# Christovis/astrild

Measured on AMD Instinct MI355X. Metric: particles/sec CIC+3D-FFT P(k) on 1024^3 grid, higher is better.
Workload: dtype f32

## Files before the change

astrild_amd/csrc/fft_tile.hip:

```cpp
#include "ast_common.h"
#include "paint_tile_geom.h"
#include <algorithm>
#include <cmath>
#include <cstring>
#include <mutex>
#include <vector>

namespace {

__device__ constexpr float kCos32[16] = {
    1.0f, 0.9807852804032304f, 0.9238795325112867f, 0.8314696123025452f, 0.7071067811865476f,
    0.5555702330196023f, 0.38268343236508984f, 0.19509032201612833f, 0.0f, -0.1950903220161282f,
    -0.3826834323650897f, -0.555570233019602f, -0.7071067811865475f, -0.8314696123025453f,
    -0.9238795325112867f, -0.9807852804032304f};
__device__ constexpr float kSin32[16] = {
    0.0f, 0.19509032201612825f, 0.3826834323650898f, 0.5555702330196022f, 0.7071067811865475f,
    0.8314696123025452f, 0.9238795325112867f, 0.9807852804032304f, 1.0f, 0.9807852804032304f,
    0.9238795325112867f, 0.8314696123025455f, 0.7071067811865476f, 0.5555702330196022f,
    0.3826834323650899f, 0.1950903220161286f};

#ifndef FFT_NT
#define FFT_NT 3
#endif
typedef float f2v __attribute__((ext_vector_type(2)));
template <bool NT>
__device__ inline float2 ld_stream(const float2* p) {
    if (NT && (FFT_NT & 1)) { const f2v v = __builtin_nontemporal_load(reinterpret_cast<const f2v*>(p)); return make_float2(v.x, v.y); }
    return *p;
}
template <bool NT>
__device__ inline void st_stream(float2* p, float2 v) {
    if (NT && (FFT_NT & 2)) __builtin_nontemporal_store(f2v{v.x, v.y}, reinterpret_cast<f2v*>(p));
    else *p = v;
}
typedef float cf2 __attribute__((ext_vector_type(2)));
__device__ inline cf2 to_cf(float2 a) { return cf2{a.x, a.y}; }
__device__ inline float2 from_cf(cf2 a) { return make_float2(a.x, a.y); }
__device__ inline cf2 cmul_cf(cf2 a, cf2 w) {
    return __builtin_elementwise_fma(a.yy, cf2{-w.y, w.x}, a.xx * w);
}
__device__ inline float2 cmul(float2 a, float2 w) { return from_cf(cmul_cf(to_cf(a), to_cf(w))); }

constexpr int bitrev(int v, int bits) {
    int r = 0;
    for (int i = 0; i < bits; ++i) r |= ((v >> i) & 1) << (bits - 1 - i);
    return r;
}
constexpr int ilog2(int v) { return v <= 1 ? 0 : 1 + ilog2(v / 2); }

template <int R>
__device__ inline void fft_reg(float2 (&vv)[R]) {
    cf2 v[R];
#pragma unroll
    for (int i = 0; i < R; ++i) v[i] = to_cf(vv[i]);
#pragma unroll
    for (int h = R / 2; h >= 1; h /= 2) {
#pragma unroll
        for (int blk = 0; blk < R; blk += 2 * h) {
#pragma unroll
            for (int j = 0; j < h; ++j) {
                const cf2 a = v[blk + j], b = v[blk + j + h];
                v[blk + j] = a + b;
                const cf2 d = a - b;
                const int t = j * (16 / h);
                if (t == 0) v[blk + j + h] = d;
                else if (t == 8) v[blk + j + h] = d.yx * cf2{1.0f, -1.0f};
                else v[blk + j + h] = cmul_cf(d, cf2{kCos32[t], -kSin32[t]});
            }
        }
    }
#pragma unroll
    for (int i = 0; i < R; ++i) vv[i] = from_cf(v[i]);
}

__device__ inline int tile_isqrt(int v) {
    return (int)__builtin_amdgcn_sqrtf((float)v + 0.5f);
}

__global__ void tile_isqrt_table_kernel(int* out, int count) {
    for (int v = blockIdx.x * blockDim.x + threadIdx.x; v < count; v += gridDim.x * blockDim.x) out[v] = tile_isqrt(v);
}

struct ShellMask { const float2* src; long long lo2, hi2; int ky0 = 0; int pass = 0;
                   size_t src_elem_stride = 0, src_batch_stride = 0; };

constexpr int SHELL_BATCH = 8;
#ifndef C2C_XCD_MODE
#define C2C_XCD_MODE 2
#endif
struct ShellBatch { int count = 0; float2* work[SHELL_BATCH]; long long lo2[SHELL_BATCH], hi2[SHELL_BATCH]; };
struct C2RBatch { int count = 0; const float2* in[SHELL_BATCH]; float* out[SHELL_BATCH]; int kmax[SHELL_BATCH]; };

struct DiscEntry { int offb; unsigned S, cumS, lohi; };
struct PackDst { float2* out = nullptr; unsigned c1_log2 = 0; unsigned nbatch = 0; float2* self_out = nullptr; unsigned self_part = ~0u; unsigned pitch = 0;
                 const DiscEntry* disc = nullptr; const unsigned short* gk = nullptr; unsigned part = 0;
                 unsigned xmajor = 0; };

template <int R1, int R2, int C, bool POWER, bool INV = false, int PACK = 0>
__global__ void __launch_bounds__(C * (R1 > R2 ? R1 : R2))
__attribute__((amdgpu_waves_per_eu((POWER || C > 16) && R1 * R2 >= 1024 ? 4 : 1, (POWER || C > 16) && R1 * R2 >= 1024 ? 4 : 8)))
strided_c2c_kernel(float2* __restrict__ data, const float2* __restrict__ tw_g, size_t elem_stride,
                   size_t ncols, size_t batch_stride, unsigned tiles_per_batch, float scale,
                   double* __restrict__ partial, const unsigned* __restrict__ edge_fall, ShellMask mask = ShellMask{nullptr, 0, 0},
                   PackDst pack = PackDst{}, ShellBatch sb = ShellBatch{}) {
    constexpr int N = R1 * R2;
    constexpr int NT = C * (R1 > R2 ? R1 : R2);
    constexpr int NB = N / 2 - 1;
    constexpr bool SPLIT = (POWER || C > 16) && R1 == R2 && N * C * sizeof(float2) > 64 * 1024;
    constexpr int YN = SPLIT ? N / 2 : N;
    extern __shared__ float2 lds[];
    float2* Y = lds;
    float2* tw = lds + YN * C;
    double* shell = reinterpret_cast<double*>(lds + YN * C + N);
    unsigned tile = blockIdx.x % tiles_per_batch, b = blockIdx.x / tiles_per_batch;
#if C2C_XCD_MODE
    if ((INV || C2C_XCD_MODE == 2) && (gridDim.x / tiles_per_batch) % 8u == 0u) {
        const unsigned xcd = blockIdx.x & 7u, slot = blockIdx.x >> 3;
        b = (slot / tiles_per_batch) * 8u + xcd;
        tile = slot % tiles_per_batch;
    }
#endif
    const size_t c0 = (size_t)tile * C;
    if (INV && sb.count > 0) {
        data = sb.work[blockIdx.y];
        mask.lo2 = sb.lo2[blockIdx.y];
        mask.hi2 = sb.hi2[blockIdx.y];
    }
    if (INV && mask.hi2 > 0) {
        const long long kb = (long long)((int)b > N / 2 ? (int)b - N : (int)b);
        const long long r2 = (long long)(c0 * c0) + (mask.pass == 0 ? kb * kb : 0);
        if (r2 >= mask.hi2) return;
    }
    const float2* disc_base = nullptr;
    unsigned disc_S = 0;
    int disc_ky = 0;
    if (!INV && POWER && pack.disc != nullptr) {
        const unsigned subb = b % R1, gk = pack.gk[pack.part * (pack.nbatch / R1) + b / R1];
        const DiscEntry e = pack.disc[(size_t)tile * R2 + gk];
        const unsigned lo = e.lohi & 255u, hi = (e.lohi >> 8) & 255u;
        if (subb - lo >= hi - lo) {
            for (int i = threadIdx.x; i < NB; i += NT) partial[((size_t)b * tiles_per_batch + tile) * NB + i] = 0.0;
            return;
        }
        disc_ky = (int)(gk * R1 + subb);
        if (pack.xmajor) {
            disc_base = data + ((long long)e.offb + (long long)(subb * 16u)) * (long long)pack.xmajor;
            disc_S = 16u;
        } else {
            disc_base = data + ((long long)e.offb + (long long)(subb * 16u));
            disc_S = e.S;
        }
    } else if (!INV && POWER && mask.hi2 > 0) {
        const long long kyi = (long long)b + mask.ky0, ky = kyi > N / 2 ? kyi - N : kyi;
        if (ky * ky + (long long)(c0 * c0) > mask.hi2) {
            for (int i = threadIdx.x; i < NB; i += NT) partial[((size_t)b * tiles_per_batch + tile) * NB + i] = 0.0;
            return;
        }
    }
    for (int i = threadIdx.x; i < N; i += NT) tw[i] = tw_g[i];
    if (POWER)
        for (int i = threadIdx.x; i <= NB; i += NT) shell[i] = 0.0;
    const int c = threadIdx.x % C, sub = threadIdx.x / C;
    const bool col_ok = (unsigned)c0 + (unsigned)c < (unsigned)ncols;
    float2 u[R2];
    {
        const bool task1 = sub < R2;
        float2 v[R1];
        const bool own = INV && mask.src != nullptr && mask.src_elem_stride != 0;
        size_t es_in = own ? mask.src_elem_stride : elem_stride;
        const float2* ubase = (INV && mask.src ? mask.src : data) + (size_t)b * (own ? mask.src_batch_stride : batch_stride);
        const int lsub = task1 ? sub : R2 - 1;
        uint32_t voff = (uint32_t)lsub * (uint32_t)es_in + min((uint32_t)c0 + (uint32_t)c, (uint32_t)ncols - 1u);
        if (POWER && !INV && disc_base != nullptr) {
            es_in = disc_S;
            ubase = disc_base;
            voff = (uint32_t)lsub * disc_S + (uint32_t)c;
        }
        if (INV && mask.hi2 > 0 && mask.pass == 1) {
            const long long c02 = (long long)(c0 * c0);
#pragma unroll
            for (int n1 = 0; n1 < R1; ++n1) {
                const int row = n1 * R2 + lsub;
                const long long ky = row > N / 2 ? row - N : row;
                v[n1] = make_float2(0.f, 0.f);
                if (ky * ky + c02 < mask.hi2) v[n1] = (ubase + (size_t)(n1 * R2) * es_in)[voff];
            }
        } else if (INV && mask.hi2 > 0) {
            const long long kyb = (long long)((int)b > N / 2 ? (int)b - N : (int)b);
            const long long r2yz = kyb * kyb + (long long)(c0 * c0);
#pragma unroll
            for (int n1 = 0; n1 < R1; ++n1) {
                const int lo = n1 * R2, hi = lo + R2 - 1;
                const long long kxmin = hi <= N / 2 ? lo : (lo >= N / 2 ? N - hi : 0);
                v[n1] = make_float2(0.f, 0.f);
                if (kxmin * kxmin + r2yz < mask.hi2) v[n1] = (ubase + (size_t)(n1 * R2) * es_in)[voff];
            }
        } else {
#pragma unroll
            for (int n1 = 0; n1 < R1; ++n1) v[n1] = ld_stream<(!INV && N >= 1024)>(ubase + (size_t)(n1 * R2) * es_in + voff);
        }
        if (INV) {
            if (mask.hi2 > 0 && mask.pass == 0) {
                const long long kz = (long long)min(c0 + c, ncols - 1), ky = (long long)((int)b > N / 2 ? (int)b - N : (int)b);
                const long long m2yz = ky * ky + kz * kz;
#pragma unroll
                for (int n1 = 0; n1 < R1; ++n1) {
                    const int row = n1 * R2 + lsub;
                    const long long kx = row > N / 2 ? row - N : row, m2 = kx * kx + m2yz;
                    if (m2 < mask.lo2 || m2 >= mask.hi2) v[n1] = make_float2(0.f, 0.f);
                }
            }
#pragma unroll
            for (int n1 = 0; n1 < R1; ++n1) v[n1].y = -v[n1].y;
        }
        fft_reg<R1>(v);
        __syncthreads();
        if (!SPLIT) {
            if (task1) {
#pragma unroll
                for (int k1 = 0; k1 < R1; ++k1) {
                    float2 y = v[bitrev(k1, ilog2(R1))];
                    if (k1 != 0) y = cmul(y, tw[sub * k1]);
                    Y[(sub * R1 + k1) * C + c] = y;
                }
            }
            __syncthreads();
            if (sub < R1) {
#pragma unroll
                for (int n2 = 0; n2 < R2; ++n2) u[n2] = Y[(n2 * R1 + sub) * C + c];
            }
        } else {
            constexpr int H = R2 / 2;
#pragma unroll
            for (int half = 0; half < 2; ++half) {
                if (sub / H == half) {
#pragma unroll
                    for (int k1 = 0; k1 < R1; ++k1) {
                        float2 y = v[bitrev(k1, ilog2(R1))];
                        if (k1 != 0) y = cmul(y, tw[sub * k1]);
                        Y[((sub - half * H) * R1 + k1) * C + c] = y;
                    }
                }
                __syncthreads();
#pragma unroll
                for (int nh = 0; nh < H; ++nh) u[half * H + nh] = Y[(nh * R1 + sub) * C + c];
                if (half == 0) __syncthreads();
            }
        }
    }
    if (sub < R1) {
        fft_reg<R2>(u);
        int tid_s = (int)threadIdx.x;
        if (C > 16) asm volatile("" : "+v"(tid_s));
        const int cs = C > 16 ? tid_s % C : c;
        const bool ok_s = C > 16 ? (unsigned)c0 + (unsigned)cs < (unsigned)ncols : col_ok;
        if (PACK == 2 && !POWER) {
            static_assert(PACK != 2 || C == 16, "the disc layout's tiles are 16 columns");
            const int4 ev = reinterpret_cast<const int4*>(pack.disc + (size_t)tile * R2)[threadIdx.x % R2];
#pragma unroll
            for (int k2 = 0; k2 < R2; ++k2) {
                float2 x = u[bitrev(k2, ilog2(R2))];
                x.x *= scale;
                x.y *= scale;
                const int offb = __builtin_amdgcn_readlane(ev.x, k2);
                const unsigned S = (unsigned)__builtin_amdgcn_readlane(ev.y, k2), cumS = (unsigned)__builtin_amdgcn_readlane(ev.z, k2);
                const unsigned lohi = (unsigned)__builtin_amdgcn_readlane(ev.w, k2);
                const unsigned lo = lohi & 255u, hi = (lohi >> 8) & 255u, part = lohi >> 16;
                if (pack.xmajor) {
                    float2* const ub = pack.self_out + ((long long)offb * (long long)pack.xmajor + (long long)(b * 16u));
                    if ((unsigned)sub - lo < hi - lo)
                        st_stream<(N >= 1024)>(ub + ((uint32_t)sub * 16u * pack.xmajor + (uint32_t)(threadIdx.x & 15u)), x);
                    continue;
                }
                float2* const ub = (part == pack.self_part ? pack.self_out : pack.out + (size_t)pack.nbatch * cumS)
                                   + ((size_t)b * S + (long long)offb);
                if ((unsigned)sub - lo < hi - lo) st_stream<(N >= 1024)>(ub + threadIdx.x, x);
            }
        } else if (ok_s && !POWER) {
            float2* const base = data + (size_t)b * batch_stride + c0 + cs;
            const int room = (!INV && mask.hi2 > 0) ? (int)mask.hi2 - (int)(c0 * c0) : 0x7fffffff;
            const int wsub0 = __builtin_amdgcn_readfirstlane((int)threadIdx.x) / C, wsub1 = wsub0 + 64 / C - 1;
#pragma unroll
            for (int k2 = 0; k2 < R2; ++k2) {
                float2 x = u[bitrev(k2, ilog2(R2))];
                x.x *= scale;
                x.y *= INV ? -scale : scale;
                if (!INV) {
                    const int aky = R1 * k2 >= N / 2 ? N - (wsub1 + R1 * k2) : wsub0 + R1 * k2;
                    if (aky * aky > room) continue;
                }
                if (PACK) {
                    const unsigned part = (unsigned)(R1 * k2) >> pack.c1_log2, r0 = (unsigned)(R1 * k2) & ((1u << pack.c1_log2) - 1u);
                    float2* const ub = part == pack.self_part
                        ? pack.self_out + ((((size_t)b) << pack.c1_log2) + r0) * pack.pitch
                        : pack.out + ((((size_t)part * pack.nbatch + b) << pack.c1_log2) + r0) * pack.pitch;
                    st_stream<(N >= 1024)>(ub + ((uint32_t)sub * pack.pitch + (uint32_t)c0 + (uint32_t)cs), x);
                } else {
                    st_stream<(!INV && N >= 1024)>(base + (size_t)(sub + R1 * k2) * elem_stride, x);
                }
            }
        }
    }
    int tid_e = (int)threadIdx.x;
    asm volatile("" : "+v"(tid_e));
    if (POWER && (unsigned)c0 + (unsigned)(tid_e % C) < (unsigned)ncols && sub < R1) {
        unsigned fallmask = 0;
        const int kyi = disc_base != nullptr ? disc_ky : (int)b + mask.ky0;
        if (edge_fall) fallmask = edge_fall[((size_t)(disc_base != nullptr ? (unsigned)disc_ky : b) * tiles_per_batch + tile) * NT + threadIdx.x];
        const int kz = (int)c0 + tid_e % C;
        const int ky = kyi > N / 2 ? kyi - N : kyi;
        const int m2yz = ky * ky + kz * kz;
        const float w = (kz > 0 && kz < N / 2) ? 2.0f : 1.0f;
#pragma unroll
        for (int k2 = 0; k2 < R2; ++k2) {
            const float2 x = u[bitrev(k2, ilog2(R2))];
            const int row = sub + R1 * k2;
            const int kx = row > N / 2 ? row - N : row;
            int sh = tile_isqrt(kx * kx + m2yz);
            sh -= (int)((fallmask >> k2) & 1u);
            if (sh >= 1 && sh <= NB) atomicAdd(&shell[sh], (double)(fmaf(x.x, x.x, x.y * x.y) * w));
        }
    }
    if (POWER) {
        __syncthreads();
        const double s2 = (double)scale * (double)scale;
        for (int i = threadIdx.x; i < NB; i += NT) partial[((size_t)b * tiles_per_batch + tile) * NB + i] = shell[i + 1] * s2;
    }
}

constexpr int REDUCE_ROWS = 1024;
__global__ void __launch_bounds__(256)
shell_partials_stage1_kernel(const double* __restrict__ partial, size_t nwg, int nb, double* __restrict__ partial2) {
    const size_t per = (nwg + REDUCE_ROWS - 1) / REDUCE_ROWS;
    const size_t g0 = (size_t)blockIdx.x * per, g1 = g0 + per < nwg ? g0 + per : nwg;
    for (int bin = threadIdx.x; bin < nb; bin += 256) {
        double acc = 0.0;
#pragma unroll 8
        for (size_t g = g0; g < g1; ++g) acc += partial[g * nb + bin];
        partial2[(size_t)blockIdx.x * nb + bin] = acc;
    }
}
__global__ void __launch_bounds__(256)
shell_partials_stage2_kernel(const double* __restrict__ partial2, int nb, double pnorm, int first_bin,
                             double* __restrict__ psum) {
    __shared__ double part[32][8];
    const int b8 = threadIdx.x & 7, grp = threadIdx.x >> 3;
    const int bin = blockIdx.x * 8 + b8;
    double acc = 0.0;
    if (bin < nb) {
#pragma unroll 8
        for (int r = grp; r < REDUCE_ROWS; r += 32) acc += partial2[(size_t)r * nb + bin];
    }
    part[grp][b8] = acc;
    __syncthreads();
    if (grp == 0 && bin < nb && bin >= first_bin) {
        double t = 0.0;
        for (int k = 0; k < 32; ++k) t += part[k][b8];
        psum[bin] += pnorm * t;
    }
}

constexpr int MLOW_FWD = 5, MBOX_FWD = MLOW_FWD + 1;
__device__ constexpr double kC16f[16] = {1.0, 0.92387953251128674, 0.70710678118654752, 0.38268343236508977, 0.0,
                                         -0.38268343236508977, -0.70710678118654752, -0.92387953251128674, -1.0,
                                         -0.92387953251128674, -0.70710678118654752, -0.38268343236508977, 0.0,
                                         0.38268343236508977, 0.70710678118654752, 0.92387953251128674};
__device__ constexpr double kS16f[16] = {0.0, -0.38268343236508977, -0.70710678118654752, -0.92387953251128674, -1.0,
                                         -0.92387953251128674, -0.70710678118654752, -0.38268343236508977, 0.0,
                                         0.38268343236508977, 0.70710678118654752, 0.92387953251128674, 1.0,
                                         0.92387953251128674, 0.70710678118654752, 0.38268343236508977};

struct SlabFold { int xb0 = 0, ntx = 0, row_lo = 0, row_hi = 0; bool ranges = false; };

template <int R1, int R2, int C, int FOLDW, bool LOWK = false>
__global__ void __launch_bounds__(C * R2)
__attribute__((amdgpu_waves_per_eu(LOWK ? 4 : 1, LOWK ? 4 : 8)))
rows_r2c_kernel(const float* __restrict__ in, float2* __restrict__ out, const float2* __restrict__ tw_g,
                size_t nrows, size_t in_pitch, size_t out_pitch, float scale, float mean,
                const float* __restrict__ rec, const double2* __restrict__ lowk_lane = nullptr,
                double* __restrict__ lowz = nullptr, SlabFold sf = SlabFold{}) {
    constexpr int M = R1 * R2, N = 2 * M;
    constexpr int NT = C * R2;
    constexpr int R2P = R2 + 1;
    constexpr int MP = M + 1;
    extern __shared__ float2 lds[];
    float2* Y = lds;
    float2* tw = lds + C * (R1 * R2P > MP ? R1 * R2P : MP);
    for (int i = threadIdx.x; i < N; i += NT) tw[i] = tw_g[i];

    const size_t row0 = (size_t)blockIdx.x * C;
    const int n2 = threadIdx.x % R2, r = threadIdx.x / R2;
    {
        const float2* zin = reinterpret_cast<const float2*>(in + min(row0 + r, nrows - 1) * in_pitch);
        float2 v[R1];
#pragma unroll
        for (int n1 = 0; n1 < R1; ++n1) v[n1] = ld_stream<(N >= 1024)>(zin + n1 * R2 + n2);
        if (FOLDW != 0) {
            constexpr int W = FOLDW != 0 ? FOLDW : 2;
            const int ng = (int)(2 * M);
            const size_t row = min(row0 + r, nrows - 1);
            const float* src[3];
            int ns;
            if (sf.ntx == 0) {
                const int xb = sf.xb0 + (int)(row / ng), trow = xb / ast::TX;
                ns = !sf.ranges || (trow >= sf.row_lo && trow < sf.row_hi)
                         ? ast::halo_sources<float, W>(rec, xb, (int)(row % ng), ng, ng / ast::TX, ng / ast::TY, src) : 0;
            } else {
                const int xb = sf.xb0 + (int)(row / ng), trow = xb / ast::TX;
                ns = trow >= sf.row_lo && trow < sf.row_hi
                         ? ast::halo_sources<float, W>(rec, xb, (int)(row % ng), ng, sf.ntx, ng / ast::TY, src, false) : 0;
            }
            if (ns > 0) {
                float2 h[R1];
#pragma unroll
                for (int n1 = 0; n1 < R1; ++n1) h[n1] = reinterpret_cast<const float2*>(src[0])[n1 * R2 + n2];
                if (ns > 1) {
#pragma unroll
                    for (int n1 = 0; n1 < R1; ++n1) {
                        const float2 t = reinterpret_cast<const float2*>(src[1])[n1 * R2 + n2];
                        h[n1].x += t.x;
                        h[n1].y += t.y;
                    }
                }
                if (ns > 2) {
#pragma unroll
                    for (int n1 = 0; n1 < R1; ++n1) {
                        const float2 t = reinterpret_cast<const float2*>(src[2])[n1 * R2 + n2];
                        h[n1].x += t.x;
                        h[n1].y += t.y;
                    }
                }
#pragma unroll
                for (int n1 = 0; n1 < R1; ++n1) {
                    v[n1].x += h[n1].x;
                    v[n1].y += h[n1].y;
                }
            }
        }
        if (LOWK) {
            static_assert(!LOWK || ((R1 == 16 || R1 == 8) && (R2 == 32 || R2 == 16) && MBOX_FWD == 6), "R1-th roots from the 16th-root table; 32 or 16 lanes per row");
            double acc[14];
#pragma unroll
            for (int e = 0; e < 14; ++e) acc[e] = 0.0;
#pragma unroll
            for (int p = 0; p < 2; ++p) {
                double f[R1];
#pragma unroll
                for (int n1 = 0; n1 < R1; ++n1) f[n1] = (double)(p ? v[n1].y : v[n1].x);
#pragma unroll
                for (int kz = 0; kz <= MBOX_FWD; ++kz) {
                    double tr = 0.0, ti = 0.0;
#pragma unroll
                    for (int n1 = 0; n1 < R1; ++n1) {
                        const int rr = ((kz * n1) % R1) * (16 / R1);
                        if (rr == 0) tr += f[n1];
                        else if (rr == 4) ti -= f[n1];
                        else if (rr == 8) tr -= f[n1];
                        else if (rr == 12) ti += f[n1];
                        else { tr = fma(f[n1], kC16f[rr], tr); ti = fma(f[n1], kS16f[rr], ti); }
                    }
                    const double2 a = lowk_lane[(n2 * (MBOX_FWD + 1) + kz) * 2 + p];
                    acc[2 * kz] = fma(a.x, tr, fma(-a.y, ti, acc[2 * kz]));
                    acc[2 * kz + 1] = fma(a.x, ti, fma(a.y, tr, acc[2 * kz + 1]));
                }
            }
            const int lane = threadIdx.x & 63;
            auto level = [&](auto count_tag, int mask) {
                constexpr int COUNT = decltype(count_tag)::value;
                const bool upper = (lane & mask) != 0;
#pragma unroll
                for (int i = 0; i < COUNT / 2; ++i) {
                    const double keep = upper ? acc[i + COUNT / 2] : acc[i];
                    const double send = upper ? acc[i] : acc[i + COUNT / 2];
                    acc[i] = keep + __shfl_xor(send, mask, 64);
                }
            };
            constexpr int TOP = R2 / 2;
            level(std::integral_constant<int, 14>{}, TOP);
            acc[7] = 0.0;
            level(std::integral_constant<int, 8>{}, TOP / 2);
            level(std::integral_constant<int, 4>{}, TOP / 4);
            level(std::integral_constant<int, 2>{}, TOP / 8);
            if (R2 == 32) acc[0] += __shfl_xor(acc[0], 1, 64);
            constexpr int SH = R2 == 32 ? 1 : 0;
            const int sel = lane >> SH;
            const int sub = ((sel >> 2) & 1) * 4 + ((sel >> 1) & 1) * 2 + (sel & 1);
            if ((R2 == 16 || (lane & 1) == 0) && sub < 7 && row0 + r < nrows)
                lowz[(row0 + r) * (size_t)(2 * (MBOX_FWD + 1)) + ((sel >> 3) & 1) * 7 + sub] = acc[0];
        }
#pragma unroll
        for (int n1 = 0; n1 < R1; ++n1) {
            v[n1].x -= mean;
            v[n1].y -= mean;
        }
        fft_reg<R1>(v);
        __syncthreads();
#pragma unroll
        for (int k1 = 0; k1 < R1; ++k1) {
            float2 y = v[bitrev(k1, ilog2(R1))];
            if (k1 != 0) y = cmul(y, tw[2 * n2 * k1]);
            Y[(r * R1 + k1) * R2P + n2] = y;
        }
    }
    __syncthreads();
    float2 u[R2];
    const int k1 = threadIdx.x % R1, r2 = threadIdx.x / R1;
    const bool task2 = r2 < C;
    if (task2) {
#pragma unroll
        for (int j = 0; j < R2; ++j) u[j] = Y[(r2 * R1 + k1) * R2P + j];
        fft_reg<R2>(u);
    }
    __syncthreads();
    if (task2) {
#pragma unroll
        for (int k2 = 0; k2 < R2; ++k2) Y[r2 * MP + k1 + R1 * k2] = u[bitrev(k2, ilog2(R2))];
    }
// ... 713 lines not shown
            if (L.part_of[k] == r) L.gk.push_back((unsigned short)k);
    L.tab.assign((size_t)L.tiles * L.nblk, DiscEntry{0, 0, 0, 0});
    L.S.assign(parts, 0);
    L.cumS.assign(parts, 0);
    for (int r = 0; r < parts; ++r) {
        unsigned rows = 0;
        for (unsigned t = 0; t < L.tiles; ++t)
            for (unsigned j = 0; j < nb; ++j) {
                const unsigned k = L.gk[(size_t)r * nb + j];
                int lo = -1, hi = -1;
                for (int sub = 0; sub < L.r1; ++sub)
                    if (disc_row_in(n, (int)(k * L.r1 + sub), t)) { if (lo < 0) lo = sub; hi = sub + 1; }
                DiscEntry& e = L.tab[(size_t)t * L.nblk + k];
                if (lo < 0) { e.lohi = (unsigned)r << 16; continue; }
                e.offb = 16 * ((int)rows - lo);
                e.lohi = (unsigned)lo | (unsigned)hi << 8 | (unsigned)r << 16;
                rows += (unsigned)(hi - lo);
            }
        L.S[r] = 16 * rows;
    }
    for (int r = 1; r < parts; ++r) L.cumS[r] = L.cumS[r - 1] + L.S[r - 1];
    for (auto& e : L.tab) { const unsigned r = e.lohi >> 16; e.S = L.S[r]; e.cumS = L.cumS[r]; }
}

struct DiscCache {
    std::mutex m;
    std::vector<DiscLayout*> all;
    const DiscLayout* get(size_t n, int parts, bool device, const DiscLayout::Dev** dv) {
        std::lock_guard<std::mutex> lock(m);
        DiscLayout* L = nullptr;
        for (auto* x : all) if (x->n == n && x->parts == parts) L = x;
        if (!L) { L = new DiscLayout; disc_build(*L, n, parts); all.push_back(L); }
        if (!device) return L;
        int dev = 0;
        if (hipGetDevice(&dev) != hipSuccess) return nullptr;
        for (auto& d : L->devs) if (d.dev == dev) { *dv = &d; return L; }
        DiscLayout::Dev d{dev, nullptr, nullptr};
        if (hipMalloc(&d.tab, L->tab.size() * sizeof(DiscEntry)) != hipSuccess) return nullptr;
        if (hipMalloc(&d.gk, L->gk.size() * sizeof(unsigned short)) != hipSuccess) return nullptr;
        if (hipMemcpy(d.tab, L->tab.data(), L->tab.size() * sizeof(DiscEntry), hipMemcpyHostToDevice) != hipSuccess) return nullptr;
        if (hipMemcpy(d.gk, L->gk.data(), L->gk.size() * sizeof(unsigned short), hipMemcpyHostToDevice) != hipSuccess) return nullptr;
        L->devs.reserve(64);
        L->devs.push_back(d);
        *dv = &L->devs.back();
        return L;
    }
} g_disc;

static bool disc_geometry_ok(size_t n, int parts) {
    return (n == 256 || n == 512 || n == 1024) && parts >= 1 && parts <= 256 && (n / tile_r1(n)) % (size_t)parts == 0;
}

}

extern "C" int ast_fft_tile_supported(int dtype, size_t n) {
    return dtype == AST_F32 && (n == 256 || n == 512 || n == 1024) ? 1 : 0;
}

extern "C" int ast_fft_tile_c2c(void* data, int dtype, size_t n, size_t elem_stride, size_t ncols, size_t batch,
                                size_t batch_stride, double scale, void* stream) {
    AST_CHECK_ARG(data != nullptr && ncols >= 1 && batch >= 1 && elem_stride >= ncols);
    AST_CHECK_ARG(ast_fft_tile_supported(dtype, n));
    const float2* tw = g_tw.get((int)n);
    if (!tw) { ast::set_error("ast_fft_tile_c2c: twiddle table allocation failed"); return AST_ERR_HIP; }
    hipStream_t s = ast::as_stream(stream);
    AST_PROF("fft_tile.c2c", s);
    return dispatch_c2c<false>(n, (float2*)data, tw, elem_stride, ncols, batch, batch_stride, (float)scale, nullptr, s);
}

extern "C" int ast_fft_tile_c2c_packed(const void* planes, void* packed, int dtype, size_t n, size_t ncols, size_t pitch,
                                       size_t nplanes, int parts, int self_part, void* self_out, double scale, void* stream) {
    AST_CHECK_ARG(planes != nullptr && planes != packed && planes != self_out && ncols >= 1 && nplanes >= 1 && pitch >= ncols);
    AST_CHECK_ARG((self_out == nullptr) || (self_part >= 0 && self_part < parts));
    AST_CHECK_ARG(packed != nullptr || (self_out != nullptr && parts == 1));
    AST_CHECK_ARG(ast_fft_tile_supported(dtype, n));
    AST_CHECK_ARG(parts >= 1 && (parts & (parts - 1)) == 0 && n % (size_t)parts == 0);
    AST_CHECK_ARG(n / (size_t)parts >= (n == 1024 ? 32u : 16u));
    AST_CHECK_ARG(pitch < (1u << 24));
    const float2* tw = g_tw.get((int)n);
    if (!tw) { ast::set_error("ast_fft_tile_c2c_packed: twiddle table allocation failed"); return AST_ERR_HIP; }
    hipStream_t s = ast::as_stream(stream);
    PackDst pack;
    pack.out = (float2*)packed;
    pack.nbatch = (unsigned)nplanes;
    pack.pitch = (unsigned)pitch;
    if (self_out) { pack.self_out = (float2*)self_out; pack.self_part = (unsigned)self_part; }
    for (size_t c1 = n / (size_t)parts; c1 > 1; c1 >>= 1) ++pack.c1_log2;
    AST_PROF("fft_tile.c2c", s);
    float2* d = (float2*)const_cast<void*>(planes);
    if (n == 1024 && pitch % 16 == 0 && getenv("AST_FFT_PACK_C32"))
        return launch_c2c_pack<32, 32, FWD_C>(d, tw, pitch, ncols, nplanes, n * pitch, (float)scale, pack, s);
    if (n == 1024) return launch_c2c_pack<32, 32, 16>(d, tw, pitch, ncols, nplanes, n * pitch, (float)scale, pack, s);
    if (n == 512) return launch_c2c_pack<16, 32, 16>(d, tw, pitch, ncols, nplanes, n * pitch, (float)scale, pack, s);
    return launch_c2c_pack<16, 16, 16>(d, tw, pitch, ncols, nplanes, n * pitch, (float)scale, pack, s);
}

__global__ void lowk_lane_kernel(double2* __restrict__ out, int n, int lanes) {
    const int i = blockIdx.x * blockDim.x + threadIdx.x;
    if (i >= lanes * 7 * 2) return;
    const int p = i & 1, kz = (i >> 1) % 7, n2 = (i >> 1) / 7;
    double sn, cs;
    sincospi(-2.0 * (double)((kz * (2 * n2 + p)) % n) / (double)n, &sn, &cs);
    out[i] = make_double2(cs, sn);
}
struct LowkLaneCache {
    std::mutex m;
// ... 177 lines not shown
    const size_t lds = (size_t)n * sizeof(double2);
    lowk_axis_kernel<<<dim3((unsigned)nx, 1), 256, lds, s>>>(lowz, n, n, 0, MBOX + 1, lowy);
    const int inner = (2 * MBOX + 1) * (MBOX + 1);
    lowk_axis_kernel<<<dim3(1, LOWK_XPARTS), 256, lds, s>>>(lowy, n, nx, x0, inner, parts);
    lowk_parts_reduce_kernel<<<(unsigned)((LOWK_MODES + 255) / 256), 256, 0, s>>>(parts, LOWK_XPARTS, (int)LOWK_MODES, accumulate, modes);
    AST_CHECK_LAUNCH();
    return AST_OK;
}

static int power_3d_impl(const void* grid, void* scratch, size_t scratch_bytes, int dtype, size_t n, double boxsize,
                         double mean, double* psum, const void* rec, int window, int lowk, int binning, void* stream) {
    AST_CHECK_ARG(grid != nullptr && scratch != nullptr && psum != nullptr && boxsize > 0.0);
    AST_CHECK_ARG(lowk == 0 || lowk == 1);
    AST_CHECK_ARG(binning == AST_BIN_INTEGER || binning == AST_BIN_FLOAT64);
    const double kf_rule = binning == AST_BIN_FLOAT64 ? 2.0 * M_PI / boxsize : 0.0;
    AST_CHECK_ARG(ast_fft_tile_supported(dtype, n));
    AST_CHECK_ARG(scratch_bytes >= ast_fft_tile_power_scratch_bytes(n));
    const size_t nz = n / 2 + 1, nzp = (nz + 15) / 16 * 16, tiles = (nz + 15) / 16;
    float2* spec = (float2*)scratch;
    float2* disc = (float2*)((char*)scratch + n * n * nzp * sizeof(float2));
    double* partial = (double*)((char*)disc + power_disc_bytes(n));
    const float2* tw = g_tw.get((int)n);
    if (!tw) { ast::set_error("ast_fft_tile_power_3d: twiddle table allocation failed"); return AST_ERR_HIP; }
    hipStream_t s = ast::as_stream(stream);
    double* lowk_sums = (double*)((char*)scratch + power_core_bytes(n)) - 64;
    const SideStream* side = nullptr;
    double2* modes = (double2*)((char*)scratch + (power_core_bytes(n) + 255) / 256 * 256);
    double2* work = (double2*)((char*)modes + (LOWK_MODES * sizeof(double2) + 255) / 256 * 256);
    const bool z_fused = lowk && !getenv("AST_LOWK_SEPARATE");
    auto lowk_rest = [&]() -> int {
        AST_CHECK_HIP(hipEventRecord(side->in, s));
        AST_CHECK_HIP(hipStreamWaitEvent(side->side, side->in, 0));
        {
            AST_PROF("fft_tile.lowk", side->side);
            int rc = lowk_modes((const float*)grid, (const float*)rec, window, (int)n, 0, (int)n, 0, modes, work, side->side, z_fused);
            if (rc != AST_OK) return rc;
            const double ng = (double)n * (double)n * (double)n;
            lowk_shell_kernel<<<1, 256, 0, side->side>>>(modes, boxsize * boxsize * boxsize / (ng * ng), kf_rule, lowk_sums);
            AST_CHECK_LAUNCH();
        }
        AST_CHECK_HIP(hipEventRecord(side->done, side->side));
        return AST_OK;
    };
    if (lowk) {
        side = g_side.get(s);
        if (!side) { ast::set_error("ast_fft_tile_power_3d: side stream creation failed"); return AST_ERR_HIP; }
        if (!z_fused) { const int rc = lowk_rest(); if (rc != AST_OK) return rc; }
    }
    int rc = rows_r2c_impl(grid, spec, dtype, n, n * n, n, nzp, 1.0, mean, stream, rec, window,
                           z_fused ? reinterpret_cast<double*>(work) : nullptr);
    if (rc != AST_OK) return rc;
    if (z_fused) { rc = lowk_rest(); if (rc != AST_OK) return rc; }
    const long long prune2 = getenv("AST_FFT_NO_PRUNE") ? 0 : (long long)(n / 2) * (long long)(n / 2);
    const double inv_ng = 1.0 / ((double)n * (double)n * (double)n);
    const char* disc_env = getenv("AST_FFT_DISC");
    const bool use_disc = prune2 != 0 && disc_env != nullptr && (disc_env[0] == '1' || disc_env[0] == '2');
    const unsigned xmajor = use_disc && disc_env[0] == '2' ? (unsigned)n : 0u;
    if (use_disc) {
        const DiscLayout::Dev* dv = nullptr;
        const DiscLayout* L = g_disc.get(n, 1, true, &dv);
        if (!L) { ast::set_error("ast_fft_tile_power_3d: disc table allocation failed"); return AST_ERR_HIP; }
        {
            AST_PROF("fft_tile.c2c", s);
            PackDst pk;
            pk.nbatch = (unsigned)n;
            pk.disc = dv->tab;
            pk.self_out = disc;
            pk.self_part = 0;
            pk.xmajor = xmajor;
            if (n == 1024) rc = launch_c2c_pack<32, 32, 16, 2>(spec, tw, nzp, nz, n, n * nzp, 1.0f, pk, s);
            else if (n == 512) rc = launch_c2c_pack<16, 32, 16, 2>(spec, tw, nzp, nz, n, n * nzp, 1.0f, pk, s);
            else rc = launch_c2c_pack<16, 16, 16, 2>(spec, tw, nzp, nz, n, n * nzp, 1.0f, pk, s);
            if (rc != AST_OK) return rc;
        }
        AST_PROF("fft_tile.c2c_power", s);
        const unsigned* edge_fall = nullptr;
        if (kf_rule != 0.0) {
            edge_fall = g_edge.get(n, boxsize, s);
            if (!edge_fall) { ast::set_error("ast_fft_tile_power_3d: edge table allocation failed"); return AST_ERR_HIP; }
        }
        PackDst src;
        src.disc = dv->tab;
        src.gk = dv->gk;
        src.nbatch = (unsigned)n;
        src.xmajor = xmajor;
        rc = dispatch_c2c<true>(n, disc, tw, xmajor ? 16 : L->S[0], nz, n, 16, (float)inv_ng, partial, s, edge_fall, 0, 0, src);
        if (rc != AST_OK) return rc;
    } else {
        {
            AST_PROF("fft_tile.c2c", s);
            rc = dispatch_c2c<false>(n, spec, tw, nzp, nz, n, n * nzp, 1.0f, nullptr, s, nullptr, 0, prune2);
            if (rc != AST_OK) return rc;
        }
        AST_PROF("fft_tile.c2c_power", s);
        const unsigned* edge_fall = nullptr;
        if (kf_rule != 0.0) {
            edge_fall = g_edge.get(n, boxsize, s);
            if (!edge_fall) { ast::set_error("ast_fft_tile_power_3d: edge table allocation failed"); return AST_ERR_HIP; }
        }
        rc = dispatch_c2c<true>(n, spec, tw, n * nzp, nz, n, nzp, (float)inv_ng, partial, s, edge_fall, 0, prune2);
        if (rc != AST_OK) return rc;
    }
    AST_PROF("fft_tile.shell_reduce", s);
    const int nb = (int)(n / 2 - 1);
    double* partial2 = (double*)scratch;
    shell_partials_stage1_kernel<<<REDUCE_ROWS, 256, 0, s>>>(partial, n * tiles, nb, partial2);
    shell_partials_stage2_kernel<<<(nb + 7) / 8, 256, 0, s>>>(partial2, nb, boxsize * boxsize * boxsize, lowk ? MLOW : 0, psum);
    if (lowk) {
        AST_CHECK_HIP(hipStreamWaitEvent(s, side->done, 0));
        lowk_patch_kernel<<<1, 64, 0, s>>>(lowk_sums, MLOW, psum);
    }
    AST_CHECK_LAUNCH();
    return AST_OK;
}

extern "C" size_t ast_lowk_work_bytes(size_t n, size_t nx) {
    return (nx * n * (MBOX + 1) + nx * (2 * MBOX + 1) * (MBOX + 1) + (size_t)LOWK_XPARTS * LOWK_MODES) * sizeof(double2);
}
extern "C" int ast_lowk_mode_count(void) { return (int)LOWK_MODES; }
extern "C" int ast_lowk_shell_count(void) { return MLOW; }

extern "C" int ast_lowk_modes(const void* planes, int dtype, size_t n, size_t x0, size_t nx, int accumulate, void* modes,
                              void* work, size_t work_bytes, void* stream) {
    AST_CHECK_ARG(planes && modes && work && nx >= 1 && x0 + nx <= n && (nx * n) % 4 == 0);
    AST_CHECK_ARG(ast_fft_tile_supported(dtype, n) || (dtype == AST_F32 && n == 2048));
    AST_CHECK_ARG(work_bytes >= ast_lowk_work_bytes(n, nx));
    hipStream_t s = ast::as_stream(stream);
    AST_PROF("fft_tile.lowk", s);
    return lowk_modes((const float*)planes, nullptr, 0, (int)n, (int)x0, (int)nx, accumulate, (double2*)modes, (double2*)work, s);
}

extern "C" int ast_lowk_modes_from_z(size_t n, size_t x0, size_t nx, int accumulate, void* modes, void* work, size_t work_bytes,
                                     void* stream) {
    AST_CHECK_ARG(modes && work && nx >= 1 && x0 + nx <= n);
    AST_CHECK_ARG(ast_fft_tile_supported(AST_F32, n));
    AST_CHECK_ARG(work_bytes >= ast_lowk_work_bytes(n, nx));
    hipStream_t s = ast::as_stream(stream);
    AST_PROF("fft_tile.lowk", s);
    return lowk_modes(nullptr, nullptr, 0, (int)n, (int)x0, (int)nx, accumulate, (double2*)modes, (double2*)work, s, true);
}

extern "C" int ast_lowk_shell_sums(const void* modes, size_t n, double boxsize, int binning, double* sums, void* stream) {
    AST_CHECK_ARG(modes && sums && boxsize > 0.0 && n >= 16);
    AST_CHECK_ARG(binning == AST_BIN_INTEGER || binning == AST_BIN_FLOAT64);
    const double ng = (double)n * (double)n * (double)n;
    lowk_shell_kernel<<<1, 256, 0, ast::as_stream(stream)>>>((const double2*)modes, boxsize * boxsize * boxsize / (ng * ng),
                                                          binning == AST_BIN_FLOAT64 ? 2.0 * M_PI / boxsize : 0.0, sums);
    AST_CHECK_LAUNCH();
    return AST_OK;
}

extern "C" int ast_fft_tile_c2r_3d(const void* spec, void* work, void* out, int dtype, size_t n, int m_lo, int m_hi,
                                   double scale, void* stream) {
    AST_CHECK_ARG(spec != nullptr && work != nullptr && out != nullptr && spec != work && work != out);
    AST_CHECK_ARG(ast_fft_tile_supported(dtype, n));
    AST_CHECK_ARG(m_lo >= 0 && (m_hi == 0 || m_hi > m_lo));
    const float2* tw = g_tw.get((int)n);
    if (!tw) { ast::set_error("ast_fft_tile_c2r_3d: twiddle table allocation failed"); return AST_ERR_HIP; }
    hipStream_t s = ast::as_stream(stream);
// ... 235 lines not shown
```

Measured before the change: 84.43 billion.

## Skip partial-zeroing for pruned tiles and handle Nyquist column separately

Pruned power-pass tiles now return without writing zeros to their partial rows, and the stage-1 shell reduction recomputes the prune condition so it skips reading those rows. By default (pruning on) the Nyquist kz column is collapsed by a dedicated reduction kernel and left out of the first c2c pass, which shrinks that pass by one column. The aim is to cut global writes and reads of unused partials and the wasted column tile, at the cost of an extra small kernel launch and a reduction test that must match the kernel's prune test exactly. Register-pinning asm and optional timestamp probes are also added, and the pinning of u is active for wide tiles.

```diff
diff --git a/astrild_amd/csrc/fft_tile.hip b/astrild_amd/csrc/fft_tile.hip
--- a/astrild_amd/csrc/fft_tile.hip
+++ b/astrild_amd/csrc/fft_tile.hip
@@ -72,6 +72,30 @@
 #pragma unroll
     for (int i = 0; i < R; ++i) vv[i] = from_cf(v[i]);
 }
+
+template <int R>
+__device__ inline void pin_regs(float2 (&a)[R]) {
+#pragma unroll
+    for (int i = 0; i < R; ++i) {
+        cf2 t = to_cf(a[i]);
+        asm volatile("" : "+v"(t));
+        a[i] = from_cf(t);
+    }
+}
+
+#ifdef FFT_STAMPS
+constexpr int FFT_STAMP_WGS = 64, FFT_STAMP_SLOTS = 8, FFT_STAMP_EVERY = 509;
+__device__ unsigned long long g_fft_stamps[FFT_STAMP_WGS * FFT_STAMP_SLOTS];
+#define FFT_STAMP(id)                                                                                                   \
+    do {                                                                                                                \
+        if (POWER && threadIdx.x == 0 && blockIdx.x % FFT_STAMP_EVERY == 7 && blockIdx.x / FFT_STAMP_EVERY < FFT_STAMP_WGS) \
+            g_fft_stamps[(blockIdx.x / FFT_STAMP_EVERY) * FFT_STAMP_SLOTS + (id)] = __builtin_amdgcn_s_memtime();         \
+    } while (0)
+#define FFT_STAMP_PIN(a) do { if (POWER) pin_regs(a); } while (0)
+#else
+#define FFT_STAMP(id) do {} while (0)
+#define FFT_STAMP_PIN(a) do {} while (0)
+#endif
 
 __device__ inline int tile_isqrt(int v) {
     return (int)__builtin_amdgcn_sqrtf((float)v + 0.5f);
@@ -152,11 +176,9 @@
         }
     } else if (!INV && POWER && mask.hi2 > 0) {
         const long long kyi = (long long)b + mask.ky0, ky = kyi > N / 2 ? kyi - N : kyi;
-        if (ky * ky + (long long)(c0 * c0) > mask.hi2) {
-            for (int i = threadIdx.x; i < NB; i += NT) partial[((size_t)b * tiles_per_batch + tile) * NB + i] = 0.0;
-            return;
-        }
-    }
+        if (ky * ky + (long long)(c0 * c0) > mask.hi2) return;
+    }
+    FFT_STAMP(0);
     for (int i = threadIdx.x; i < N; i += NT) tw[i] = tw_g[i];
     if (POWER)
         for (int i = threadIdx.x; i <= NB; i += NT) shell[i] = 0.0;
@@ -213,7 +235,10 @@
 #pragma unroll
             for (int n1 = 0; n1 < R1; ++n1) v[n1].y = -v[n1].y;
         }
+        FFT_STAMP(1);
         fft_reg<R1>(v);
+        FFT_STAMP_PIN(v);
+        FFT_STAMP(2);
         __syncthreads();
         if (!SPLIT) {
             if (task1) {
@@ -249,9 +274,16 @@
         }
     }
     if (sub < R1) {
+        FFT_STAMP_PIN(u);
+        FFT_STAMP(3);
         fft_reg<R2>(u);
+        FFT_STAMP_PIN(u);
+        FFT_STAMP(4);
         int tid_s = (int)threadIdx.x;
-        if (C > 16) asm volatile("" : "+v"(tid_s));
+        if (C > 16) {
+            asm volatile("" : "+v"(tid_s));
+            pin_regs(u);
+        }
         const int cs = C > 16 ? tid_s % C : c;
         const bool ok_s = C > 16 ? (unsigned)c0 + (unsigned)cs < (unsigned)ncols : col_ok;
         if (PACK == 2 && !POWER) {
@@ -323,22 +355,62 @@
     }
     if (POWER) {
         __syncthreads();
+        FFT_STAMP(5);
         const double s2 = (double)scale * (double)scale;
         for (int i = threadIdx.x; i < NB; i += NT) partial[((size_t)b * tiles_per_batch + tile) * NB + i] = shell[i + 1] * s2;
+        FFT_STAMP(6);
     }
 }
 
 constexpr int REDUCE_ROWS = 1024;
 __global__ void __launch_bounds__(256)
-shell_partials_stage1_kernel(const double* __restrict__ partial, size_t nwg, int nb, double* __restrict__ partial2) {
+shell_partials_stage1_kernel(const double* __restrict__ partial, size_t nwg, int nb, double* __restrict__ partial2,
+                             unsigned tiles = 1, int n = 0, long long prune2 = 0) {
     const size_t per = (nwg + REDUCE_ROWS - 1) / REDUCE_ROWS;
     const size_t g0 = (size_t)blockIdx.x * per, g1 = g0 + per < nwg ? g0 + per : nwg;
     for (int bin = threadIdx.x; bin < nb; bin += 256) {
         double acc = 0.0;
+        if (prune2 > 0) {
+            for (size_t g = g0; g < g1; g += 8) {
+                double v[8];
+#pragma unroll
+                for (int j = 0; j < 8; ++j) {
+                    const unsigned gj = (unsigned)g + (unsigned)j;
+                    const int kyi = (int)(gj / tiles), ky = kyi > n / 2 ? kyi - n : kyi, kz0 = (int)(gj % tiles) * 16;
+                    v[j] = 0.0;
+                    if (gj < (unsigned)g1 && (long long)(ky * ky + kz0 * kz0) <= prune2) v[j] = partial[(size_t)gj * nb + bin];
+                }
+#pragma unroll
+                for (int j = 0; j < 8; ++j) acc += v[j];
+            }
+        } else {
 #pragma unroll 8
-        for (size_t g = g0; g < g1; ++g) acc += partial[g * nb + bin];
+            for (size_t g = g0; g < g1; ++g) acc += partial[g * nb + bin];
+        }
         partial2[(size_t)blockIdx.x * nb + bin] = acc;
     }
+}
+
+__global__ void __launch_bounds__(256)
+nyquist_column_kernel(float2* __restrict__ spec, int n, size_t pitch) {
+    __shared__ double2 part[256];
+    float2* const col = spec + (size_t)blockIdx.x * (size_t)n * pitch + (size_t)(n / 2);
+    double2 acc = make_double2(0.0, 0.0);
+    for (int y = threadIdx.x; y < n; y += 256) {
+        const float2 v = col[(size_t)y * pitch];
+        acc.x += (double)v.x;
+        acc.y += (double)v.y;
+    }
+    part[threadIdx.x] = acc;
+    __syncthreads();
+    for (int h = 128; h >= 1; h /= 2) {
+        if ((int)threadIdx.x < h) {
+            part[threadIdx.x].x += part[threadIdx.x + h].x;
+            part[threadIdx.x].y += part[threadIdx.x + h].y;
+        }
+        __syncthreads();
+    }
+    if (threadIdx.x == 0) col[0] = make_float2((float)part[0].x, (float)part[0].y);
 }
 __global__ void __launch_bounds__(256)
 shell_partials_stage2_kernel(const double* __restrict__ partial2, int nb, double pnorm, int first_bin,
@@ -1282,6 +1354,16 @@
 }
 
 }
+
+#ifdef FFT_STAMPS
+extern "C" int ast_debug_fft_stamps(unsigned long long* stamps_host) {
+    AST_CHECK_HIP(hipDeviceSynchronize());
+    AST_CHECK_HIP(hipMemcpyFromSymbol(stamps_host, HIP_SYMBOL(g_fft_stamps), sizeof(unsigned long long) * FFT_STAMP_WGS * FFT_STAMP_SLOTS));
+    const unsigned long long zero[FFT_STAMP_WGS * FFT_STAMP_SLOTS] = {0};
+    AST_CHECK_HIP(hipMemcpyToSymbol(HIP_SYMBOL(g_fft_stamps), zero, sizeof(zero)));
+    return AST_OK;
+}
+#endif
 
 extern "C" int ast_fft_tile_supported(int dtype, size_t n) {
     return dtype == AST_F32 && (n == 256 || n == 512 || n == 1024) ? 1 : 0;
@@ -1565,6 +1647,8 @@
     if (rc != AST_OK) return rc;
     if (z_fused) { rc = lowk_rest(); if (rc != AST_OK) return rc; }
     const long long prune2 = getenv("AST_FFT_NO_PRUNE") ? 0 : (long long)(n / 2) * (long long)(n / 2);
+    const char* nyq_env = getenv("AST_FFT_NYQ_TILE");
+    const bool nyq_tile = prune2 == 0 || (nyq_env != nullptr && nyq_env[0] == '1');
     const double inv_ng = 1.0 / ((double)n * (double)n * (double)n);
     const char* disc_env = getenv("AST_FFT_DISC");
     const bool use_disc = prune2 != 0 && disc_env != nullptr && (disc_env[0] == '1' || disc_env[0] == '2');
@@ -1600,9 +1684,14 @@
         rc = dispatch_c2c<true>(n, disc, tw, xmajor ? 16 : L->S[0], nz, n, 16, (float)inv_ng, partial, s, edge_fall, 0, 0, src);
         if (rc != AST_OK) return rc;
     } else {
+        if (!nyq_tile) {
+            AST_PROF("fft_tile.nyq_col", s);
+            nyquist_column_kernel<<<(unsigned)n, 256, 0, s>>>(spec, (int)n, nzp);
+            AST_CHECK_LAUNCH();
+        }
         {
             AST_PROF("fft_tile.c2c", s);
-            rc = dispatch_c2c<false>(n, spec, tw, nzp, nz, n, n * nzp, 1.0f, nullptr, s, nullptr, 0, prune2);
+            rc = dispatch_c2c<false>(n, spec, tw, nzp, nyq_tile ? nz : nz - 1, n, n * nzp, 1.0f, nullptr, s, nullptr, 0, prune2);
             if (rc != AST_OK) return rc;
         }
         AST_PROF("fft_tile.c2c_power", s);
@@ -1617,7 +1706,7 @@
     AST_PROF("fft_tile.shell_reduce", s);
     const int nb = (int)(n / 2 - 1);
     double* partial2 = (double*)scratch;
-    shell_partials_stage1_kernel<<<REDUCE_ROWS, 256, 0, s>>>(partial, n * tiles, nb, partial2);
+    shell_partials_stage1_kernel<<<REDUCE_ROWS, 256, 0, s>>>(partial, n * tiles, nb, partial2, (unsigned)tiles, (int)n, use_disc ? 0 : prune2);
     shell_partials_stage2_kernel<<<(nb + 7) / 8, 256, 0, s>>>(partial2, nb, boxsize * boxsize * boxsize, lowk ? MLOW : 0, psum);
     if (lowk) {
         AST_CHECK_HIP(hipStreamWaitEvent(s, side->done, 0));
```

Result: no change. 84.96 billion, median of 6 (+0.6%).

## Use radix-2 real DFT and twiddle recurrence in low-k fold path

Applied to the files above, without the earlier changes.

Replaces the direct per-kz DFT sum in the low-k accumulation with a factored real 8/16-point DFT that computes only the first seven modes. Per-mode lane twiddles are now derived from one loaded twiddle by repeated complex multiplication instead of being loaded for each kz. Halo-source reads are also made streaming loads, their address lookup is moved ahead of the main row load, and the single-source case is special-cased. This cuts double-precision FLOPs and global loads in the rows_r2c kernel, at the cost of some rounding from the twiddle recurrence and a fixed emit order.

```diff
diff --git a/astrild_amd/csrc/fft_tile.hip b/astrild_amd/csrc/fft_tile.hip
--- a/astrild_amd/csrc/fft_tile.hip
+++ b/astrild_amd/csrc/fft_tile.hip
@@ -370,6 +370,61 @@
                                          0.38268343236508977, 0.70710678118654752, 0.92387953251128674, 1.0,
                                          0.92387953251128674, 0.70710678118654752, 0.38268343236508977};
 
+__device__ inline void real_dft8_low5(const double (&e)[8], double (&er)[5], double (&ei)[5]) {
+    const double a0 = e[0] + e[4], a1 = e[1] + e[5], a2 = e[2] + e[6], a3 = e[3] + e[7];
+    const double b0 = e[0] - e[4], b1 = e[1] - e[5], b2 = e[2] - e[6], b3 = e[3] - e[7];
+    const double s02 = a0 + a2, s13 = a1 + a3;
+    er[0] = s02 + s13;
+    ei[0] = 0.0;
+    er[4] = s02 - s13;
+    ei[4] = 0.0;
+    er[2] = a0 - a2;
+    ei[2] = a3 - a1;
+    const double pc = kC16f[2] * (b1 - b3), qc = kC16f[2] * (b1 + b3);
+    er[1] = b0 + pc;
+    ei[1] = -b2 - qc;
+    er[3] = b0 - pc;
+    ei[3] = b2 - qc;
+}
+template <int R1, typename Emit>
+__device__ inline void real_dft_low7(const double (&f)[R1], Emit&& emit) {
+    static_assert(R1 == 16 || R1 == 8, "16- or 8-point transform");
+    double er[5], ei[5];
+    if constexpr (R1 == 8) {
+        real_dft8_low5(f, er, ei);
+        emit(1, er[1], ei[1]);
+        emit(3, er[3], ei[3]);
+        emit(5, er[3], -ei[3]);
+        emit(0, er[0], ei[0]);
+        emit(2, er[2], ei[2]);
+        emit(4, er[4], ei[4]);
+        emit(6, er[2], -ei[2]);
+    } else {
+        double d[8], e[8];
+#pragma unroll
+        for (int j = 0; j < 8; ++j) {
+            d[j] = f[j] - f[j + 8];
+            e[j] = f[j] + f[j + 8];
+        }
+        double g[4], s[4];
+#pragma unroll
+        for (int j = 1; j < 4; ++j) { g[j] = d[j] - d[8 - j]; s[j] = d[j] + d[8 - j]; }
+#pragma unroll
+        for (int k = 1; k < 6; k += 2) {
+            double xr = d[0], xi = (k & 2) ? d[4] : -d[4];
+#pragma unroll
+            for (int j = 1; j < 4; ++j) {
+                xr = fma(g[j], kC16f[(j * k) % 16], xr);
+                xi = fma(s[j], kS16f[(j * k) % 16], xi);
+            }
+            emit(k, xr, xi);
+        }
+        real_dft8_low5(e, er, ei);
+#pragma unroll
+        for (int m = 0; m < 4; ++m) emit(2 * m, er[m], ei[m]);
+    }
+}
+
 struct SlabFold { int xb0 = 0, ntx = 0, row_lo = 0, row_hi = 0; bool ranges = false; };
 
 template <int R1, int R2, int C, int FOLDW, bool LOWK = false>
@@ -393,14 +448,12 @@
     {
         const float2* zin = reinterpret_cast<const float2*>(in + min(row0 + r, nrows - 1) * in_pitch);
         float2 v[R1];
-#pragma unroll
-        for (int n1 = 0; n1 < R1; ++n1) v[n1] = ld_stream<(N >= 1024)>(zin + n1 * R2 + n2);
+        const float* src[3];
+        int ns = 0;
         if (FOLDW != 0) {
             constexpr int W = FOLDW != 0 ? FOLDW : 2;
             const int ng = (int)(2 * M);
             const size_t row = min(row0 + r, nrows - 1);
-            const float* src[3];
-            int ns;
             if (sf.ntx == 0) {
                 const int xb = sf.xb0 + (int)(row / ng), trow = xb / ast::TX;
                 ns = !sf.ranges || (trow >= sf.row_lo && trow < sf.row_hi)
@@ -410,26 +463,36 @@
                 ns = trow >= sf.row_lo && trow < sf.row_hi
                          ? ast::halo_sources<float, W>(rec, xb, (int)(row % ng), ng, sf.ntx, ng / ast::TY, src, false) : 0;
             }
-            if (ns > 0) {
+        }
+#pragma unroll
+        for (int n1 = 0; n1 < R1; ++n1) v[n1] = ld_stream<(N >= 1024)>(zin + n1 * R2 + n2);
+        if (FOLDW != 0 && ns > 0) {
+            auto rec_ld = [&](int s, int n1) { return ld_stream<(N >= 1024)>(reinterpret_cast<const float2*>(src[s]) + n1 * R2 + n2); };
+            if (ns == 1) {
+#pragma unroll
+                for (int n1 = 0; n1 < R1; ++n1) {
+                    const float2 t = rec_ld(0, n1);
+                    v[n1].x += t.x;
+                    v[n1].y += t.y;
+                }
+            } else {
                 float2 h[R1];
 #pragma unroll
-                for (int n1 = 0; n1 < R1; ++n1) h[n1] = reinterpret_cast<const float2*>(src[0])[n1 * R2 + n2];
-                if (ns > 1) {
+                for (int n1 = 0; n1 < R1; ++n1) h[n1] = rec_ld(0, n1);
+#pragma unroll
+                for (int n1 = 0; n1 < R1; ++n1) {
+                    const float2 t = rec_ld(1, n1);
+                    h[n1].x += t.x;
+                    h[n1].y += t.y;
+                }
+                if (ns > 2) {
 #pragma unroll
                     for (int n1 = 0; n1 < R1; ++n1) {
-                        const float2 t = reinterpret_cast<const float2*>(src[1])[n1 * R2 + n2];
+                        const float2 t = rec_ld(2, n1);
                         h[n1].x += t.x;
                         h[n1].y += t.y;
                     }
                 }
-                if (ns > 2) {
-#pragma unroll
-                    for (int n1 = 0; n1 < R1; ++n1) {
-                        const float2 t = reinterpret_cast<const float2*>(src[2])[n1 * R2 + n2];
-                        h[n1].x += t.x;
-                        h[n1].y += t.y;
-                    }
-                }
 #pragma unroll
                 for (int n1 = 0; n1 < R1; ++n1) {
                     v[n1].x += h[n1].x;
@@ -439,6 +502,7 @@
         }
         if (LOWK) {
             static_assert(!LOWK || ((R1 == 16 || R1 == 8) && (R2 == 32 || R2 == 16) && MBOX_FWD == 6), "R1-th roots from the 16th-root table; 32 or 16 lanes per row");
+            const double2 la = lowk_lane[(n2 * (MBOX_FWD + 1) + 1) * 2], lb = lowk_lane[(n2 * (MBOX_FWD + 1) + 1) * 2 + 1];
             double acc[14];
 #pragma unroll
             for (int e = 0; e < 14; ++e) acc[e] = 0.0;
@@ -447,22 +511,16 @@
                 double f[R1];
 #pragma unroll
                 for (int n1 = 0; n1 < R1; ++n1) f[n1] = (double)(p ? v[n1].y : v[n1].x);
-#pragma unroll
-                for (int kz = 0; kz <= MBOX_FWD; ++kz) {
-                    double tr = 0.0, ti = 0.0;
-#pragma unroll
-                    for (int n1 = 0; n1 < R1; ++n1) {
-                        const int rr = ((kz * n1) % R1) * (16 / R1);
-                        if (rr == 0) tr += f[n1];
-                        else if (rr == 4) ti -= f[n1];
-                        else if (rr == 8) tr -= f[n1];
-                        else if (rr == 12) ti += f[n1];
-                        else { tr = fma(f[n1], kC16f[rr], tr); ti = fma(f[n1], kS16f[rr], ti); }
-                    }
-                    const double2 a = lowk_lane[(n2 * (MBOX_FWD + 1) + kz) * 2 + p];
+                const double2 base = p ? lb : la;
+                const double2 sq = make_double2(fma(base.x, base.x, -(base.y * base.y)), 2.0 * (base.x * base.y));
+                double2 a = base;
+                real_dft_low7<R1>(f, [&](int kz, double tr, double ti) __attribute__((always_inline)) {
+                    if (kz == 0) { acc[0] += tr; return; }
+                    if (kz == 2) a = sq;
+                    else if (kz != 1) a = make_double2(fma(a.x, sq.x, -(a.y * sq.y)), fma(a.x, sq.y, a.y * sq.x));
                     acc[2 * kz] = fma(a.x, tr, fma(-a.y, ti, acc[2 * kz]));
                     acc[2 * kz + 1] = fma(a.x, ti, fma(a.y, tr, acc[2 * kz + 1]));
-                }
+                });
             }
             const int lane = threadIdx.x & 63;
             auto level = [&](auto count_tag, int mask) {
```

New measurement: 83.24 billion before, 84.49 billion after (median of 6 runs). 1.01x the previous value.
